# TAMUparametric/PPOPT

Measured on NVIDIA B200. Metric: candidate active sets/sec, higher is better.
Workload: dtype f64

## Files before the change

ppopt_b200/csrc/api.cu:

```cuda
#include <cstdio>
#include <cstdlib>
#include <cstring>
#include <mutex>
#include <string>
#include <vector>

#include "../../include/ppgpu.h"
#include "common.cuh"
#include "host_math.hpp"
#include "launch.h"

using namespace ppgpu;

static thread_local std::string g_err;

struct ppgpu_program {
    ReducedProgram host;
    DevProgram dev;
    int device = 0;
    int sm_count = 0;
    std::vector<void*> allocs;
    unsigned long long* d_counters = nullptr;
    unsigned long long* d_queue = nullptr;
    int queue_slot = 0;
// ... 291 lines not shown
    if (stages & 2) {
        ProfScope ps(p, st, 1);
        e = launch_k2(p->dev, d_masks, n, d_status, next_queue(p, st), p->d_counters, p->sm_count, st);
        if (e != cudaSuccess) return fail("K2 feasibility", e);
        p->launches++;
        if (p->dev.warm_count) {
            if ((e = launch_clear_bits(d_status, n, PPG_ST_PRE, st)) != cudaSuccess) return fail("status clean-up", e);
            p->launches++;
        }
    }
    if (stages & 4) {
        ProfScope ps(p, st, 2);
        if (p->dev.is_qp && p->dev.use_gram) {
            e = launch_k34(p->dev, d_masks, n, k_act, d_status, next_queue(p, st), p->d_counters, p->sm_count, st);
            if (k_act >= 1 && k_act <= 8) p->launches++;
        } else {
            e = launch_mark_general(p->dev, n, k_act, d_status, st);
        }
        if (e != cudaSuccess) return fail("K3/K4 optimality screen", e);
        p->launches++;
    }
    return 0;
}

int ppgpu_level_eval(ppgpu_program* p, const uint64_t* d_masks, int64_t n, int32_t k_act, uint8_t* d_status,
                     int32_t stages, ppgpu_stream stream) {
    return ppgpu_level_eval_w(p, d_masks, n, k_act, d_status, stages, nullptr, nullptr, 0, nullptr, nullptr, stream);
}

int ppgpu_level_eval_w(ppgpu_program* p, const uint64_t* d_masks, int64_t n, int32_t k_act, uint8_t* d_status,
                       int32_t stages, uint64_t* d_witness, const uint64_t* d_parent_feas, int64_t parent_nf,
                       const void* d_parent_ws, const uint64_t* d_parent_wit, ppgpu_stream stream) {
    if (!p) return fail_msg("null argument");
    if (n <= 0) return 0;
    WitnessIo wio;
    wio.parent_feas = d_parent_feas; wio.parent_nf = parent_nf; wio.parent_ws = d_parent_ws; wio.parent_wit = d_parent_wit;
    const bool walk = (stages & 2) && !(stages & 8) && k_act >= 1 && p->dev.wk_ok && p->k2w_min >= 0 && n >= p->k2w_min;
    const long long chunk = walk ? walk_chunk() : level_chunk();
    for (int64_t off = 0; off < n; off += chunk) {
        const int64_t nn = n - off < chunk ? n - off : chunk;
        wio.out = d_witness ? d_witness + (size_t)off * PPGPU_WITNESS_SLOTS * p->dev.W : nullptr;
        const int rc = level_eval_chunk(p, d_masks + (size_t)off * p->dev.W, nn, k_act, d_status + off, stages,
                                        (cudaStream_t)stream, wio);
        if (rc) return rc;
    }
    return 0;
}

size_t ppgpu_scan_workspace_bytes(int64_t n) { return scan_workspace_bytes(n); }
size_t ppgpu_select_workspace_bytes(int64_t n) { return select_workspace_bytes(n); }

int ppgpu_level_select(ppgpu_program* p, const uint8_t* d_status, int64_t n, uint8_t bits, uint8_t value,
                       int64_t* d_idx_out, int64_t* h_count, void* d_ws, size_t ws_bytes, ppgpu_stream stream) {
    if (!p || !h_count) return fail_msg("null argument");
    *h_count = 0;
    if (n <= 0) return 0;
    cudaStream_t st = (cudaStream_t)stream;
    if (ws_bytes < select_workspace_bytes(n)) return fail_msg("workspace too small");
    long long* d_count = (long long*)d_ws + (select_workspace_bytes(n) / sizeof(long long) - 1);
    cudaError_t e;
    {
        ProfScope ps(p, st, 6);
        e = select_indices(d_status, n, bits, value, (long long*)d_idx_out, d_count, d_ws, ws_bytes - sizeof(long long), st);
    }
    if (e != cudaSuccess) return fail("select", e);
    p->launches += 5;
    long long cnt = 0;
    e = cudaMemcpyAsync(&cnt, d_count, sizeof(long long), cudaMemcpyDeviceToHost, st);
    if (e == cudaSuccess) e = cudaStreamSynchronize(st);
    if (e != cudaSuccess) return fail("select count", e);
    *h_count = cnt;
    return 0;
}

int ppgpu_regions_emit(ppgpu_program* p, const uint64_t* d_masks, const int64_t* d_sel, int64_t n_sel, int32_t k_act,
                       double* d_laws, double* d_rows, int32_t* d_flags, double* d_info, uint8_t* d_status,
                       ppgpu_stream stream) {
    if (!p) return fail_msg("null argument");
    if (n_sel <= 0) return 0;
    cudaError_t e;
    {
        ProfScope ps(p, (cudaStream_t)stream, 3);
        e = launch_k5(p->dev, d_masks, (const long long*)d_sel, n_sel, k_act, d_laws, d_rows, d_flags, d_info, d_status,
                      p->d_counters, p->sm_count, (cudaStream_t)stream);
    }
    if (e != cudaSuccess) return fail("K5 emit", e);
    p->launches++;
    return 0;
}

int ppgpu_children_count(ppgpu_program* p, const uint64_t* d_masks, const int64_t* d_feas_idx, int64_t nf,
                         int32_t k_act, uint64_t* d_feas_masks, uint64_t* d_survive, int64_t* d_offsets,
                         int64_t* h_total, void* d_ws, size_t ws_bytes, ppgpu_stream stream) {
    if (!p || !h_total) return fail_msg("null argument");
    *h_total = 0;
    if (nf <= 0) return 0;
    cudaStream_t st = (cudaStream_t)stream;
    cudaError_t e;
    {
        ProfScope ps(p, st, 4);
        e = children_count(p->dev, d_masks, (const long long*)d_feas_idx, nf, k_act, d_feas_masks, d_survive,
                           (long long*)d_offsets, d_ws, ws_bytes, p->d_counters, st);
    }
    if (e != cudaSuccess) return fail("K6 count", e);
    p->launches += 12;
    long long tot = 0, disorder = 0;
    e = cudaMemcpyAsync(&tot, (long long*)d_offsets + nf, sizeof(long long), cudaMemcpyDeviceToHost, st);
    if (e == cudaSuccess) e = cudaMemcpyAsync(&disorder, children_order_flag(d_ws, nf), sizeof(long long), cudaMemcpyDeviceToHost, st);
    if (e == cudaSuccess) e = cudaStreamSynchronize(st);
    if (e != cudaSuccess) return fail("K6 total", e);
    if (disorder) return fail_msg("K6: the feasible parents are not one level's sets in lexicographic order");
    *h_total = tot;
    return 0;
}

int ppgpu_children_prepare(ppgpu_program* p, const uint64_t* d_masks, const int64_t* d_feas_idx, int64_t nf,
                           uint64_t* d_feas_masks, void* d_ws, size_t ws_bytes, ppgpu_stream stream) {
    if (!p) return fail_msg("null argument");
    if (nf <= 0) return 0;
    cudaError_t e;
    {
        ProfScope ps(p, (cudaStream_t)stream, 4);
        e = children_prepare(p->dev, d_masks, (const long long*)d_feas_idx, nf, d_feas_masks, d_ws, ws_bytes, (cudaStream_t)stream);
    }
    if (e != cudaSuccess) return fail("K6 prepare", e);
    p->launches += 8;
    return 0;
}

int ppgpu_children_count_range(ppgpu_program* p, const uint64_t* d_feas_masks, int64_t nf, int32_t k_act,
                               uint64_t* d_survive, int64_t* d_counts, int64_t p_lo, int64_t p_hi, void* d_ws,
                               size_t ws_bytes, ppgpu_stream stream) {
    if (!p) return fail_msg("null argument");
    if (p_lo < 0 || p_hi > nf || p_lo > p_hi) return fail_msg("parent range outside [0, nf]");
    if (nf <= 0 || p_hi == p_lo) return 0;
    if (ws_bytes < scan_workspace_bytes(nf)) return fail_msg("workspace too small");
    cudaError_t e;
    {
        ProfScope ps(p, (cudaStream_t)stream, 4);
        e = children_count_range(p->dev, d_feas_masks, nf, k_act, d_survive, (long long*)d_counts, p_lo, p_hi, d_ws,
                                 p->d_counters, (cudaStream_t)stream);
    }
    if (e != cudaSuccess) return fail("K6 count", e);
    p->launches++;
    return 0;
}

int ppgpu_children_scan(ppgpu_program* p, int64_t* d_counts_to_offsets, int64_t nf, int64_t* h_total, void* d_ws,
                        size_t ws_bytes, ppgpu_stream stream) {
    if (!p || !h_total) return fail_msg("null argument");
    *h_total = 0;
    if (nf <= 0) return 0;
    if (ws_bytes < scan_workspace_bytes(nf)) return fail_msg("workspace too small");
    cudaStream_t st = (cudaStream_t)stream;
    cudaError_t e;
    {
        ProfScope ps(p, st, 4);
        e = children_scan((long long*)d_counts_to_offsets, nf, d_ws, st);
    }
    if (e != cudaSuccess) return fail("K6 scan", e);
    p->launches += 2;
    long long tot = 0, disorder = 0;
    e = cudaMemcpyAsync(&tot, (long long*)d_counts_to_offsets + nf, sizeof(long long), cudaMemcpyDeviceToHost, st);
    if (e == cudaSuccess) e = cudaMemcpyAsync(&disorder, children_order_flag(d_ws, nf), sizeof(long long), cudaMemcpyDeviceToHost, st);
    if (e == cudaSuccess) e = cudaStreamSynchronize(st);
    if (e != cudaSuccess) return fail("K6 total", e);
    if (disorder) return fail_msg("K6: the feasible parents are not one level's sets in lexicographic order");
    *h_total = tot;
    return 0;
}
// ... 128 lines not shown
```

ppopt_b200/csrc/k34c_compact.cu:

```cuda
#include "common.cuh"
#include "launch.h"
#include "lp_core.cuh"

#include <cstdlib>

namespace ppgpu {

struct K4cOut { int code; double beta; int pivots; long long work; };

__device__ __forceinline__ double k4c_rcp(double x) {
    double r;
    asm("rcp.approx.ftz.f64 %0, %1;" : "=d"(r) : "d"(x));
    r = r * fma(-x, r, 2.0);
    return r * fma(-x, r, 2.0);
}

__device__ __noinline__ K4cOut k4c_solve(double* __restrict__ Tab, unsigned char* __restrict__ flag, int* __restrict__ bvar,
                                         double* __restrict__ alpha, int* __restrict__ kind, int* __restrict__ nbv,
                                         double* __restrict__ prow, int m, int t, int lds, double thr, int lane) {
    const int nc = t + 1;
    const int ld = nc + 1;
    K4cOut out; out.code = PPG_LP_OPTIMAL; out.beta = -CUDART_INF; out.pivots = 0; out.work = 0;
    int live = 0;
    #pragma unroll 1
    for (int i = lane; i < m; i += 32) { bvar[i] = ld + i; live += flag[i] ? 1 : 0; }
    live = __reduce_add_sync(PPG_FULL, live);
    #pragma unroll 1
    for (int c = lane; c < ld; c += 32) { alpha[c] = 0.0; kind[c] = (c >= 1) ? 1 : 0; nbv[c] = c; }
    __syncwarp();
    double beta = 0.0;
    int degen = 0; bool bland = false;
    const int cap = 50 * (m + nc) + 200;
    for (int it = 0;; ++it) {
        int j, l; double dir = 1.0;
        if (it == 0) {
            double mn = CUDART_INF; int r0 = 0x7fffffff;
            #pragma unroll 1
            for (int i = lane; i < m; i += 32)
                if (flag[i]) { const double v = Tab[(size_t)i * lds]; if (v < mn) { mn = v; r0 = i; } }
            warp_argmin(mn, r0);
            if (r0 == 0x7fffffff) { out.code = PPG_LP_UNBOUNDED; out.beta = CUDART_INF; return out; }
            j = nc; l = r0;
            if (lane == 0) alpha[nc] = -1.0;
            __syncwarp();
        } else {
            out.beta = beta;
            if (beta >= thr) { out.code = PPG_LP_EARLY; return out; }
            if (it > cap) { out.code = PPG_LP_ITERLIM; return out; }
            double sc = 0.0; int key = 0x7fffffff, jc = 0x7fffffff;
            #pragma unroll 1
            for (int c = 1 + lane; c < ld; c += 32) {
                const double a = alpha[c];
                const double s2 = kind[c] == 1 ? fabs(a) : (kind[c] == 2 ? -a : 0.0);
                if (s2 > PPG_OPT_TOL) {
                    if (!bland) { if (s2 > sc) { sc = s2; jc = c; } }
                    else if (nbv[c] < key) { key = nbv[c]; jc = c; sc = s2; }
                }
            }
            if (!__any_sync(PPG_FULL, jc != 0x7fffffff)) { out.code = PPG_LP_OPTIMAL; return out; }
            if (!bland) {
                const double ws = warp_max_nonneg(sc);
                j = __reduce_min_sync(PPG_FULL, (jc != 0x7fffffff && sc == ws) ? jc : 0x7fffffff);
            } else {
                const int wk = __reduce_min_sync(PPG_FULL, key);
                j = __reduce_min_sync(PPG_FULL, key == wk ? jc : 0x7fffffff);
            }
            const double aj = alpha[j];
            const bool entering_free = kind[j] == 1;
            dir = (entering_free && aj > 0.0) ? -1.0 : 1.0;
            double hb = CUDART_INF;
            #pragma unroll 1
            for (int i = lane; i < m; i += 32) {
                if (!flag[i]) continue;
                const double cv = dir * Tab[(size_t)i * lds + j];
                if (cv > PPG_TINY) {
                    const double rhs = fmax(Tab[(size_t)i * lds], 0.0);
                    hb = fmin(hb, (rhs + PPG_HARRIS) * k4c_rcp(cv));
                }
            }
            hb = warp_min_nonneg(hb);
            if (hb == CUDART_INF) { out.code = PPG_LP_UNBOUNDED; out.beta = CUDART_INF; return out; }
            double lp = 0.0, lr = CUDART_INF; int lrow = 0x7fffffff, lb = 0x7fffffff;
            #pragma unroll 1
            for (int i = lane; i < m; i += 32) {
                if (!flag[i]) continue;
                const double cv = dir * Tab[(size_t)i * lds + j];
                if (cv > PPG_TINY) {
                    const double rat = fmax(Tab[(size_t)i * lds], 0.0) * k4c_rcp(cv);
                    if (rat <= hb) {
                        const bool better = bland ? (bvar[i] < lb) : (cv > lp);
                        if (better) { lp = cv; lrow = i; lb = bvar[i]; lr = rat; }
                    }
                }
            }
            if (bland) {
                const int wb = __reduce_min_sync(PPG_FULL, lb);
                l = __reduce_min_sync(PPG_FULL, lb == wb ? lrow : 0x7fffffff);
            } else {
                const double wp = warp_max_nonneg(lp);
                l = __reduce_min_sync(PPG_FULL, (lrow != 0x7fffffff && lp == wp) ? lrow : 0x7fffffff);
            }
            if (l == 0x7fffffff) { out.code = PPG_LP_UNBOUNDED; out.beta = CUDART_INF; return out; }
            const double gr = __shfl_sync(PPG_FULL, lr, l & 31);
            if (gr <= PPG_DEGEN_STEP) { if (++degen > PPG_BLAND_AFTER) bland = true; } else degen = 0;
        }
        const bool entering_free = kind[j] == 1;
        double* Tl = Tab + (size_t)l * lds;
        const double inv = k4c_rcp(Tl[j]);
        __syncwarp();
        #pragma unroll 1
        for (int c = lane; c < ld; c += 32) prow[c] = (c == j) ? 0.0 : Tl[c] * inv;
        __syncwarp();
        const double aj = alpha[j];
        #pragma unroll 1
        for (int i = lane; i < m; i += 32) {
            if (!flag[i] || i == l) continue;
            double* Ti = Tab + (size_t)i * lds;
            const double col = Ti[j];
            if (col != 0.0) {
                #pragma unroll 1
                for (int c = 0; c < ld; ++c) Ti[c] = fma(-col, prow[c], Ti[c]);
                Ti[j] = -col * inv;
            }
            if (Ti[0] < 0.0 && Ti[0] > -1e-9) Ti[0] = 0.0;
        }
        __syncwarp();
        beta = fma(-aj, prow[0], beta);
        #pragma unroll 1
        for (int c = 1 + lane; c < ld; c += 32) alpha[c] = (c == j) ? -aj * inv : fma(-aj, prow[c], alpha[c]);
        #pragma unroll 1
        for (int c = lane; c < ld; c += 32) Tl[c] = (c == j) ? inv : prow[c];
        out.pivots++; out.work += (long long)live * (nc + 1);
        if (lane == 0) {
            const int leave_var = bvar[l], enter_var = nbv[j];
            kind[j] = 2; nbv[j] = leave_var;
            if (entering_free) flag[l] = 0; else bvar[l] = enter_var;
        }
        if (entering_free) live--;
        __syncwarp();
    }
}

__global__ void __launch_bounds__(128)
k34c_kernel(DevProgram P, const uint64_t* __restrict__ masks, long long n, int k_act, uint8_t* __restrict__ status,
            unsigned long long* __restrict__ queue, unsigned long long* __restrict__ counters, int use_pre, int warp_bytes,
            int lds) {
    extern __shared__ unsigned char k34c_smem[];
    const int warp = threadIdx.x >> 5, lane = threadIdx.x & 31;
    const int t = P.t, t1 = P.t + 1, mi = P.mi, W = P.W, k = k_act, m = P.R0;
    unsigned char* base = k34c_smem + (size_t)warp * warp_bytes;
    double* Tab = reinterpret_cast<double*>(base); base += (size_t)m * lds * 8;
    double* S = reinterpret_cast<double*>(base); base += (size_t)k * k * 8;
    double* Lam = reinterpret_cast<double*>(base); base += (size_t)k * t1 * 8;
    double* alpha = reinterpret_cast<double*>(base); base += (size_t)lds * 8;
    double* prow = reinterpret_cast<double*>(base); base += (size_t)lds * 8;
    int* act = reinterpret_cast<int*>(base); base += (size_t)((k + 1) & ~1) * 4;
    int* bvar = reinterpret_cast<int*>(base); base += (size_t)((m + 1) & ~1) * 4;
    int* kind = reinterpret_cast<int*>(base); base += (size_t)((lds + 1) & ~1) * 4;
    int* nbv = reinterpret_cast<int*>(base); base += (size_t)((lds + 1) & ~1) * 4;
    unsigned char* flag = base;
    unsigned long long n_lp = 0, n_piv = 0, n_work = 0, n_num = 0;
    const long long nblocks = (n + 31) / 32;
    for (;;) {
        unsigned long long v = 0;
        if (lane == 0) v = atomicAdd(queue, 1ull);
        const long long item = (long long)__shfl_sync(PPG_FULL, v, 0);
        if (item >= nblocks) break;
        const long long c0 = item * 32 + lane;
        const uint8_t sb = c0 < n ? status[c0] : 0;
        unsigned todo = __ballot_sync(PPG_FULL, (sb & PPG_ST_FEAS) && (!use_pre || (sb & PPG_ST_PRE)));
        while (todo) {
            const int src = __ffs((int)todo) - 1;
            todo &= todo - 1u;
            const long long idx = item * 32 + src;
            uint8_t st = (uint8_t)__shfl_sync(PPG_FULL, (int)sb, src);
            if (use_pre) st &= (uint8_t)~PPG_ST_PRE;
            const uint64_t* mk = masks + idx * W;
            __syncwarp();
            #pragma unroll 1
            for (int j = lane; j < k; j += 32) act[j] = mask_nth(mk, W, j);
            __syncwarp();
            #pragma unroll 1
            for (int e = lane; e < k * k; e += 32) {
                const int a = e / k, b2 = e - a * k;
                S[e] = __ldg(P.G + (size_t)act[a] * mi + act[b2]);
            }
            __syncwarp();
            bool pd = true;
            #pragma unroll 1
            for (int j = 0; j < k; ++j) {
                const double d = S[j * k + j];
                if (!(d > 0.0)) { pd = false; break; }
                const double sd = sqrt(d);
                __syncwarp();
                #pragma unroll 1
                for (int i = j + 1 + lane; i < k; i += 32) S[i * k + j] /= sd;
                if (lane == 0) S[j * k + j] = sd;
                __syncwarp();
                #pragma unroll 1
                for (int i = j + 1 + lane; i < k; i += 32) {
                    const double lij = S[i * k + j];
                    #pragma unroll 1
                    for (int c = j + 1; c <= i; ++c) S[i * k + c] = fma(-lij, S[c * k + j], S[i * k + c]);
                }
                __syncwarp();
            }
            bool pass = false, numeric = false, thin = false;
            if (!pd) {
                numeric = true;
            } else {
                if (lane < t1) {
                    #pragma unroll 1
                    for (int i = 0; i < k; ++i) {
                        double s = -__ldg(P.V + (size_t)act[i] * t1 + lane);
                        #pragma unroll 1
                        for (int j = 0; j < i; ++j) s = fma(-S[i * k + j], Lam[j * t1 + lane], s);
                        Lam[i * t1 + lane] = s / S[i * k + i];
                    }
                    #pragma unroll 1
                    for (int i = k - 1; i >= 0; --i) {
                        double s = Lam[i * t1 + lane];
                        #pragma unroll 1
                        for (int j = i + 1; j < k; ++j) s = fma(-S[j * k + i], Lam[j * t1 + lane], s);
                        Lam[i * t1 + lane] = s / S[i * k + i];
                    }
                }
                __syncwarp();
                bool reject = false;
                #pragma unroll 1
                for (int j = lane; j < k; j += 32) {
                    double ub = Lam[j * t1], mx = 0.0, mag = fabs(Lam[j * t1]);
                    #pragma unroll 1
                    for (int c = 0; c < t; ++c) {
                        const double a = Lam[j * t1 + 1 + c];
                        const double lo = __ldg(P.th_lo + c), hi = __ldg(P.th_hi + c);
                        mx = fmax(mx, fabs(a));
                        if (a != 0.0) { const double term = fmax(a * lo, a * hi); ub += term; mag += fabs(term); }
                    }
                    if (mx > PPG_ZERO_ROW) { if (ub < -1e-9 * fmax(1.0, mag)) reject = true; }
                    else if (mx <= PPG_ZERO_ROW && Lam[j * t1] < -PPG_FEAS_TOL) reject = true;
                }
                if (__any_sync(PPG_FULL, reject)) {
                    if (use_pre && lane == 0) status[idx] = st;
                    continue;
                }
                bool zero_viol = false;
                double lo1 = -CUDART_INF, hi1 = CUDART_INF;
                #pragma unroll 1
                for (int row = lane; row < m; row += 32) {
                    double* T = Tab + (size_t)row * lds;
                    if (row < mi) {
                        if (mask_test(mk, row)) {
                            const int pos = mask_rank(mk, row);
                            T[0] = Lam[pos * t1];
                            #pragma unroll 1
                            for (int c = 1; c < t1; ++c) T[c] = -Lam[pos * t1 + c];
                        } else {
// ... 4 lines not shown
                                const double g = __ldg(P.G + (size_t)act[a] * mi + row);
                                #pragma unroll 1
                                for (int c = 0; c < t1; ++c) T[c] = fma(g, Lam[a * t1 + c], T[c]);
                            }
                            #pragma unroll 1
                            for (int c = 1; c < t1; ++c) T[c] = -T[c];
                        }
                    } else {
                        const int o = row - mi;
                        T[0] = __ldg(P.b_t + o);
                        #pragma unroll 1
                        for (int c = 1; c < t1; ++c) T[c] = __ldg(P.A_t + (size_t)o * t + c - 1);
                    }
                    double mx = 0.0, nn = 0.0;
                    #pragma unroll 1
                    for (int c = 1; c < t1; ++c) { mx = fmax(mx, fabs(T[c])); nn = fma(T[c], T[c], nn); }
                    unsigned char fl = 0;
                    if (!(mx <= PPG_ZERO_ROW)) {
                        const double inv = 1.0 / sqrt(nn);
                        #pragma unroll 1
                        for (int c = 0; c < t1; ++c) T[c] *= inv;
                        T[t1] = 1.0;
                        fl = 1;
                        if (t == 1) { const double q = T[0] / T[1]; if (T[1] > 0.0) hi1 = fmin(hi1, q); else lo1 = fmax(lo1, q); }
                    } else if (T[0] < -PPG_FEAS_TOL) {
                        zero_viol = true;
                    }
                    flag[row] = fl;
                }
                __syncwarp();
                if (!__any_sync(PPG_FULL, zero_viol)) {
                    if (t == 1) {
#pragma unroll
                        for (int o = 16; o > 0; o >>= 1) {
                            lo1 = fmax(lo1, shfl_xor_d(lo1, o));
                            hi1 = fmin(hi1, shfl_xor_d(hi1, o));
                        }
                        pass = (lo1 + 0.5 * PPG_WIDTH_1D <= hi1);
                    } else {
                        const K4cOut res = k4c_solve(Tab, flag, bvar, alpha, kind, nbv, prow, m, t, lds, PPG_RADIUS_SCREEN, lane);
                        pass = res.code == PPG_LP_EARLY || (res.code == PPG_LP_OPTIMAL && res.beta >= PPG_RADIUS_SCREEN);
                        thin = res.code == PPG_LP_OPTIMAL && !pass && res.beta >= -PPG_RADIUS_BAND;
                        if (res.code == PPG_LP_ITERLIM) numeric = true;
                        n_lp++; n_piv += res.pivots; n_work += (unsigned long long)res.work;
                    }
                }
            }
            if (lane == 0) {
                uint8_t s2 = st;
                if (pass) s2 |= PPG_ST_OPT;
                if (thin) s2 |= PPG_ST_THIN;
                if (numeric) { s2 |= PPG_ST_NUMERIC; n_num++; }
                if (s2 != st || use_pre) status[idx] = s2;
            }
        }
    }
    if (lane == 0 && (n_lp || n_num)) {
        atomicAdd(&counters[CNT_K4_LPS], n_lp);
        atomicAdd(&counters[CNT_K4_PIVOTS], n_piv);
        atomicAdd(&counters[CNT_K4_WORK], n_work);
        if (n_num) atomicAdd(&counters[CNT_NUMERIC], n_num);
    }
}

cudaError_t launch_k34_compact(const DevProgram& P, const uint64_t* masks, long long n, int k_act, uint8_t* status,
                               unsigned long long* queue, unsigned long long* counters, int sm_count, cudaStream_t st,
                               int use_pre, bool* handled) {
    *handled = false;
    static const int on = getenv("PPGPU_K34_COMPACT") ? atoi(getenv("PPGPU_K34_COMPACT")) : 1;
    if (!on) return cudaSuccess;
    constexpr int WPC = 4;
    const int m = P.R0, t1 = P.t + 1, ld = P.t + 2, lds = ld | 1, k = k_act;
    size_t wb = (size_t)m * lds * 8 + (size_t)k * k * 8 + (size_t)k * t1 * 8 + (size_t)2 * lds * 8 +
                (size_t)(((k + 1) & ~1) + ((m + 1) & ~1) + 2 * ((lds + 1) & ~1)) * 4 + (size_t)m;
    wb = (wb + 15) & ~(size_t)15;
    const size_t smem = wb * WPC;
    if (smem > 200 * 1024) return cudaSuccess;
    cudaError_t e = allow_max_smem(k34c_kernel);
    if (e != cudaSuccess) return e;
    int occ = 0;
    e = cudaOccupancyMaxActiveBlocksPerMultiprocessor(&occ, k34c_kernel, 32 * WPC, smem);
    if (e != cudaSuccess) return e;
    if (occ < 1) occ = 1;
    long long grid = (long long)sm_count * occ;
    const long long need = (n + 32 * WPC - 1) / (32 * WPC);
    if (grid > need) grid = need;
    if (grid < 1) grid = 1;
    k34c_kernel<<<(unsigned)grid, 32 * WPC, smem, st>>>(P, masks, n, k_act, status, queue, counters, use_pre, (int)wb, lds);
    *handled = true;
    return cudaGetLastError();
}

__global__ void __launch_bounds__(128)
cheb_batch_kernel(const double* __restrict__ rows, const long long* __restrict__ row_off, long long n_poly, int t,
                  double* __restrict__ radius, int* __restrict__ code, int warp_bytes, int lds, int max_rows) {
    extern __shared__ unsigned char cheb_smem[];
    const int warp = threadIdx.x >> 5, lane = threadIdx.x & 31, t1 = t + 1;
    unsigned char* base = cheb_smem + (size_t)warp * warp_bytes;
    double* Tab = reinterpret_cast<double*>(base); base += (size_t)max_rows * lds * 8;
    double* alpha = reinterpret_cast<double*>(base); base += (size_t)lds * 8;
    double* prow = reinterpret_cast<double*>(base); base += (size_t)lds * 8;
    int* bvar = reinterpret_cast<int*>(base); base += (size_t)((max_rows + 1) & ~1) * 4;
    int* kind = reinterpret_cast<int*>(base); base += (size_t)((lds + 1) & ~1) * 4;
    int* nbv = reinterpret_cast<int*>(base); base += (size_t)((lds + 1) & ~1) * 4;
    unsigned char* flag = base;
    for (long long p = (long long)blockIdx.x * (blockDim.x >> 5) + warp; p < n_poly; p += (long long)gridDim.x * (blockDim.x >> 5)) {
        const long long r0 = row_off[p];
        const int m = (int)(row_off[p + 1] - r0);
        bool bad = false;
        __syncwarp();
#pragma unroll 1
        for (int i = lane; i < m; i += 32) {
            const double* src = rows + (size_t)(r0 + i) * t1;
            double* T = Tab + (size_t)i * lds;
            double nn = 0.0;
            T[0] = src[0];
#pragma unroll 1
            for (int c = 1; c < t1; ++c) { T[c] = src[c]; nn = fma(src[c], src[c], nn); }
            T[t1] = sqrt(nn);
            flag[i] = nn > 0.0 ? 1 : 0;
            if (!(nn > 0.0) && src[0] < 0.0) bad = true;
        }
        __syncwarp();
        K4cOut res; res.code = PPG_LP_INFEAS_EQ; res.beta = -CUDART_INF;
        if (!__any_sync(PPG_FULL, bad) && m > 0)
            res = k4c_solve(Tab, flag, bvar, alpha, kind, nbv, prow, m, t, lds, CUDART_INF, lane);
        if (lane == 0) { radius[p] = res.beta; code[p] = res.code; }
    }
}

cudaError_t launch_cheb_batch(const double* rows, const long long* row_off, long long n_poly, int t, int max_rows,
                              double* radius, int* code, int sm_count, cudaStream_t st) {
    constexpr int WPC = 4;
    const int ld = t + 2, lds = ld | 1;
    size_t wb = (size_t)max_rows * lds * 8 + (size_t)2 * lds * 8 + (size_t)(((max_rows + 1) & ~1) + 2 * ((lds + 1) & ~1)) * 4 +
                (size_t)max_rows;
    wb = (wb + 15) & ~(size_t)15;
    const size_t smem = wb * WPC;
    if (smem > 200 * 1024) return cudaErrorInvalidValue;
    cudaError_t e = allow_max_smem(cheb_batch_kernel);
    if (e != cudaSuccess) return e;
    long long grid = (n_poly + WPC - 1) / WPC;
    if (grid > (long long)sm_count * 4) grid = (long long)sm_count * 4;
    if (grid < 1) return cudaSuccess;
    cheb_batch_kernel<<<(unsigned)grid, 32 * WPC, smem, st>>>(rows, row_off, n_poly, t, radius, code, (int)wb, lds, max_rows);
    return cudaGetLastError();
}

}
```

ppopt_b200/csrc/k5_emit.cu:

```cuda
#include "common.cuh"
#include "launch.h"
#include "lp_core.cuh"

namespace ppgpu {

constexpr int K5_WARPS = 4;
constexpr int K5_THREADS = K5_WARPS * 32;

template <int RPT, int DC>
__global__ void __launch_bounds__(K5_THREADS)
k5_emit_kernel(DevProgram P, const uint64_t* __restrict__ masks, const long long* __restrict__ sel, long long n_sel,
               int k_act, double* __restrict__ laws_out, double* __restrict__ rows_out, int32_t* __restrict__ flags_out,
               double* __restrict__ info_out, uint8_t* __restrict__ status, unsigned long long* __restrict__ counters) {
    typedef LpCore<1, RPT, DC> Core;
    extern __shared__ double dyn_smem[];
    __shared__ typename Core::Shared sh_all[K5_WARPS];
    __shared__ double red_v[K5_WARPS];
    __shared__ int red_i[K5_WARPS];
    __shared__ double s_info[4];
    __shared__ int s_ok;
    __shared__ int s_full;
    __shared__ int s_thin;
    const int tid = threadIdx.x, warp = tid >> 5, lane = tid & 31;
    const int n = P.n, t = P.t, t1 = P.t + 1, m = P.m, ne = P.ne, mi = P.mi, R0 = P.R0, W = P.W;
    const int k = ne + k_act, N = n + k, ld = N + t1;
    double* M = dyn_smem;
    double* rows = M + (size_t)N * ld;
    int* flags = reinterpret_cast<int*>(rows + (size_t)R0 * t1);
    int* actf = flags + R0;
    int* keptf = actf + k;
    unsigned long long n_lp = 0, n_piv = 0, n_work = 0;

    for (long long si = blockIdx.x; si < n_sel; si += gridDim.x) {
        const long long idx = sel[si];
        const uint64_t* mk = masks + idx * W;
        __syncthreads();
        for (int j = tid; j < k; j += K5_THREADS) actf[j] = j < ne ? j : ne + mask_nth(mk, W, j - ne);
        if (tid == 0) { s_ok = 1; s_full = 0; s_thin = 0; s_info[0] = 0.0; s_info[1] = -CUDART_INF; s_info[2] = -CUDART_INF; s_info[3] = CUDART_INF; }
        __syncthreads();
        for (int e = tid; e < N * ld; e += K5_THREADS) {
            const int r = e / ld, c = e - r * ld;
            double v = 0.0;
            if (r < k) {
                const int row = actf[r];
                if (c < n) v = __ldg(P.A + (size_t)row * n + c);
                else if (c == N) v = __ldg(P.b + row);
                else if (c > N) v = __ldg(P.F + (size_t)row * t + (c - N - 1));
            } else {
                const int i = r - k;
                if (c < n) v = __ldg(P.Q + (size_t)i * n + c);
                else if (c < N) v = __ldg(P.A + (size_t)actf[c - n] * n + i);
                else if (c == N) v = -__ldg(P.c + i);
                else v = -__ldg(P.H + (size_t)i * t + (c - N - 1));
            }
            M[e] = v;
        }
        __syncthreads();
        for (int col = 0; col < N; ++col) {
            double best = -1.0; int p = 0x7fffffff;
            for (int i = col + tid; i < N; i += K5_THREADS) {
                const double a = fabs(M[(size_t)i * ld + col]);
                if (a > best) { best = a; p = i; }
            }
            warp_argmax(best, p);
            if (lane == 0) { red_v[warp] = best; red_i[warp] = p; }
            __syncthreads();
            best = red_v[0]; p = red_i[0];
#pragma unroll
            for (int w = 1; w < K5_WARPS; ++w)
                if (red_v[w] > best || (red_v[w] == best && red_i[w] < p)) { best = red_v[w]; p = red_i[w]; }
            if (!(best > 0.0) || !isfinite(best)) { if (tid == 0) s_ok = 0; __syncthreads(); break; }
            if (p != col) {
                for (int c = tid; c < ld; c += K5_THREADS) {
                    const double a = M[(size_t)p * ld + c];
                    M[(size_t)p * ld + c] = M[(size_t)col * ld + c];
                    M[(size_t)col * ld + c] = a;
                }
            }
            __syncthreads();
            const double inv = 1.0 / M[(size_t)col * ld + col];
            __syncthreads();
            for (int i = col + 1 + tid; i < N; i += K5_THREADS) M[(size_t)i * ld + col] *= inv;
            __syncthreads();
            const int tw = ld - col - 1, th = N - col - 1;
            for (int e = tid; e < tw * th; e += K5_THREADS) {
                const int i = col + 1 + e / tw, c = col + 1 + e % tw;
                M[(size_t)i * ld + c] = fma(-M[(size_t)i * ld + col], M[(size_t)col * ld + c], M[(size_t)i * ld + c]);
            }
            __syncthreads();
        }
        __syncthreads();
        const bool singular = s_ok == 0;
// ... 77 lines not shown
            if (warp == 0) {
                if (t == 1) {
                    double lo = -CUDART_INF, hi = CUDART_INF;
                    for (int r = lane; r < R0; r += 32)
                        if (flags[r] & 1) {
                            const double q = rows[(size_t)r * 2] / rows[(size_t)r * 2 + 1];
                            if (rows[(size_t)r * 2 + 1] > 0.0) hi = fmin(hi, q); else lo = fmax(lo, q);
                        }
#pragma unroll
                    for (int o = 16; o > 0; o >>= 1) {
                        lo = fmax(lo, shfl_xor_d(lo, o));
                        hi = fmin(hi, shfl_xor_d(hi, o));
                    }
                    if (lane == 0) {
                        s_info[1] = 0.5 * (hi - lo); s_info[2] = lo; s_info[3] = hi;
                        s_full = (lo + PPG_WIDTH_1D <= hi) ? 1 : 0;
                    }
                } else {
                    double rad_lo = -CUDART_INF, rad_hi = -CUDART_INF;
                    int code = PPG_LP_OPTIMAL;
                    for (int attempt = 0; attempt < 2; ++attempt) {
                        double T[RPT][DC];
                        int rflag[RPT], bv[RPT];
                        static_for<RPT>([&](auto RR) {
                            constexpr int rr = decltype(RR)::value;
                            const int row = rr * 32 + lane;
                            const bool on = row < R0 && (flags[row] & 1);
#pragma unroll
                            for (int c = 0; c < DC; ++c) T[rr][c] = (on && c < t1) ? rows[(size_t)row * t1 + c] : ((on && c == t1) ? 1.0 : 0.0);
                            rflag[rr] = on ? 1 : 0;
                            bv[rr] = 0;
                        });
                        const double thr = attempt == 0 ? PPG_RADIUS + PPG_RADIUS_BAND : CUDART_INF;
                        LpOut res = Core::solve(sh_all[0], T, rflag, R0, t1, thr, true, lane, true, &bv);
                        n_lp++; n_piv += res.pivots; n_work += (unsigned long long)res.work;
                        code = res.code;
                        rad_hi = res.beta;
                        if (code != PPG_LP_EARLY && code != PPG_LP_OPTIMAL) break;
                        double* th = &sh_all[0].P[0][0][0];
                        __syncwarp();
                        if (lane < t) th[lane] = 0.0;
                        __syncwarp();
                        static_for<RPT>([&](auto RR) {
                            constexpr int rr = decltype(RR)::value;
                            if (rflag[rr] == 3) {
                                const int c = bv[rr] < 0 ? -bv[rr] : bv[rr];
                                if (c >= 1 && c <= t) th[c - 1] = bv[rr] < 0 ? -T[rr][0] : T[rr][0];
                            }
                        });
                        __syncwarp();
                        double lo = CUDART_INF;
                        for (int r = lane; r < R0; r += 32)
                            if (flags[r] & 1) {
                                double sl = rows[(size_t)r * t1];
                                for (int c = 0; c < t; ++c) sl = fma(-rows[(size_t)r * t1 + 1 + c], th[c], sl);
                                lo = fmin(lo, sl);
                            }
#pragma unroll
                        for (int o = 16; o > 0; o >>= 1) lo = fmin(lo, shfl_xor_d(lo, o));
                        rad_lo = lo;
                        __syncwarp();
                        if (code == PPG_LP_OPTIMAL || rad_lo > PPG_RADIUS + PPG_RADIUS_BAND) break;
                    }
                    const bool solved = code == PPG_LP_EARLY || code == PPG_LP_OPTIMAL;
                    const bool ok = solved && rad_lo > PPG_RADIUS;
                    if (lane == 0) {
                        s_info[1] = solved ? rad_lo : rad_hi;
                        s_full = ok ? 1 : 0;
                        s_thin = (solved && rad_hi >= -PPG_RADIUS_BAND && rad_lo <= PPG_RADIUS + PPG_RADIUS_BAND) ? 1 : 0;
                    }
                }
            }
            __syncthreads();
            region = s_full != 0;
        }
        if (region) {
            if (t == 1) {
                const double lo = s_info[2], hi = s_info[3];
                for (int r = tid; r < R0; r += K5_THREADS)
                    if (flags[r] & 1) {
                        const double q = rows[(size_t)r * 2] / rows[(size_t)r * 2 + 1];
                        if (lo <= q && q <= hi) keptf[r] = 1;
                    }
            } else {
                for (int a = warp; a < R0; a += K5_WARPS) {
                    if (!(flags[a] & 1)) continue;
                    double T[RPT][DC];
                    int rflag[RPT];
                    static_for<RPT>([&](auto RR) {
                        constexpr int rr = decltype(RR)::value;
                        const int row = rr * 32 + lane;
                        const bool on = row < R0 && (flags[row] & 1);
#pragma unroll
                        for (int c = 0; c < DC; ++c)
                            T[rr][c] = (on && c < t1) ? rows[(size_t)row * t1 + c] : ((on && c == t1 && row != a) ? 1.0 : 0.0);
                        rflag[rr] = on ? (row == a ? 2 : 1) : 0;
                    });
                    LpOut res = Core::solve(sh_all[warp], T, rflag, R0, t1, -PPG_REDUND_TOL, false, lane);
                    n_lp++; n_piv += res.pivots; n_work += (unsigned long long)res.work;
                    const bool feas = res.code == PPG_LP_EARLY || res.code == PPG_LP_UNBOUNDED ||
                                      (res.code == PPG_LP_OPTIMAL && res.beta >= -PPG_REDUND_TOL);
                    if (lane == 0 && feas) keptf[a] = 1;
                }
            }
            __syncthreads();
            for (int r = tid; r < R0; r += K5_THREADS) if (keptf[r]) flags[r] |= 2;
            __syncthreads();
            if (t != 1) {
                for (int i = tid; i < R0; i += K5_THREADS) {
                    bool dup = false;
                    if ((flags[i] & 3) == 3) {
                        for (int j = 0; j < i && !dup; ++j) {
                            if ((flags[j] & 3) != 3) continue;
                            bool same = true;
                            for (int c = 0; c < t1 && same; ++c) same = rows[(size_t)i * t1 + c] == rows[(size_t)j * t1 + c];
                            dup = same;
                        }
                    }
                    keptf[i] = dup ? 1 : 0;
                }
                __syncthreads();
                for (int r = tid; r < R0; r += K5_THREADS) if (keptf[r]) flags[r] |= 4;
            }
            __syncthreads();
        }
        for (int e = tid; e < R0 * t1; e += K5_THREADS) rows_out[(size_t)si * R0 * t1 + e] = singular ? 0.0 : rows[e];
        for (int r = tid; r < R0; r += K5_THREADS) flags_out[(size_t)si * R0 + r] = singular ? 0 : flags[r];
        if (tid == 0) {
            info_out[si * 4 + 0] = region ? 1.0 : (singular ? -1.0 : 0.0);
            info_out[si * 4 + 1] = s_info[1];
            info_out[si * 4 + 2] = s_info[2];
            info_out[si * 4 + 3] = s_info[3];
            uint8_t st = status[idx];
            if (region) st |= PPG_ST_REGION;
            if (s_thin && !singular) st |= PPG_ST_THIN;
            if (singular) st |= PPG_ST_NUMERIC;
            status[idx] = st;
        }
    }
    if (lane == 0 && n_lp) {
        atomicAdd(&counters[CNT_K5_LPS], n_lp);
        atomicAdd(&counters[CNT_K5_PIVOTS], n_piv);
        atomicAdd(&counters[CNT_K5_WORK], n_work);
    }
}

template <int RPT, int DC>
static cudaError_t launch_k5_t(const DevProgram& P, const uint64_t* masks, const long long* idx, long long n_sel, int k_act,
                               double* laws, double* rows, int32_t* flags, double* info, uint8_t* status,
                               unsigned long long* counters, int sm_count, cudaStream_t st) {
    auto kern = k5_emit_kernel<RPT, DC>;
    const int k = P.ne + k_act, N = P.n + k, ld = N + P.t + 1;
    const size_t smem = ((size_t)N * ld + (size_t)P.R0 * (P.t + 1)) * sizeof(double) + (size_t)(2 * P.R0 + k + 2) * sizeof(int);
    if (smem > 200 * 1024) return cudaErrorInvalidValue;
    cudaError_t e;
    if ((e = fit_smem(kern, smem)) != cudaSuccess) return e;
    long long grid = n_sel;
    const long long cap = (long long)sm_count * 8;
    if (grid > cap) grid = cap;
    if (grid < 1) return cudaSuccess;
    kern<<<(unsigned)grid, K5_THREADS, smem, st>>>(P, masks, idx, n_sel, k_act, laws, rows, flags, info, status, counters);
    return cudaGetLastError();
}

#define K5_RPT_SWITCH(DCV)                                                                                                            \
    if (P.R0 <= 32) return launch_k5_t<1, DCV>(P, masks, idx, n_sel, k_act, laws, rows, flags, info, status, counters, sm_count, st);  \
    if (P.R0 <= 64) return launch_k5_t<2, DCV>(P, masks, idx, n_sel, k_act, laws, rows, flags, info, status, counters, sm_count, st);  \
    if (P.R0 <= 128) return launch_k5_t<4, DCV>(P, masks, idx, n_sel, k_act, laws, rows, flags, info, status, counters, sm_count, st); \
    if (P.R0 <= 256) return launch_k5_t<8, DCV>(P, masks, idx, n_sel, k_act, laws, rows, flags, info, status, counters, sm_count, st); \
    return cudaErrorInvalidValue;

cudaError_t launch_k5(const DevProgram& P, const uint64_t* masks, const long long* idx, long long n_sel, int k_act,
                      double* laws, double* rows, int32_t* flags, double* info, uint8_t* status,
                      unsigned long long* counters, int sm_count, cudaStream_t st) {
    if (P.t + 2 <= 8) { K5_RPT_SWITCH(8) }
    if (P.t + 2 <= 16) { K5_RPT_SWITCH(16) }
    return cudaErrorInvalidValue;
}

}
```

ppopt_b200/csrc/launch.h:

```cpp
#pragma once
#include <cuda_runtime.h>
#include <stdint.h>

#include "common.cuh"

namespace ppgpu {

template <class K>
inline cudaError_t allow_max_smem(K kern) {
    int dev = 0, lim = 0;
    cudaError_t e = cudaGetDevice(&dev);
    if (e == cudaSuccess) e = cudaDeviceGetAttribute(&lim, cudaDevAttrMaxSharedMemoryPerBlockOptin, dev);
    if (e != cudaSuccess) return e;
    cudaFuncAttributes fa;
    if ((e = cudaFuncGetAttributes(&fa, kern)) != cudaSuccess) return e;
    return cudaFuncSetAttribute(kern, cudaFuncAttributeMaxDynamicSharedMemorySize, lim - (int)fa.sharedSizeBytes);
}

template <class K>
inline cudaError_t fit_smem(K kern, size_t dyn) {
    cudaFuncAttributes fa;
    const cudaError_t e = cudaFuncGetAttributes(&fa, kern);
    if (e != cudaSuccess) return e;
    return fa.sharedSizeBytes + dyn > 48 * 1024 ? allow_max_smem(kern) : cudaSuccess;
}

int k2_pad_columns(int ncols_with_rhs);

cudaError_t launch_k1(const DevProgram& P, const uint64_t* masks, long long n, int k_act, uint8_t* status,
                      unsigned long long* counters, int sm_count, cudaStream_t st);
cudaError_t launch_k2(const DevProgram& P, const uint64_t* masks, long long n, uint8_t* status,
                      unsigned long long* queue, unsigned long long* counters, int sm_count, cudaStream_t st);
cudaError_t launch_k2a(const DevProgram& P, const uint64_t* masks, long long n, int k_act, uint8_t* status,
                       unsigned long long* queue, unsigned long long* counters, int max_iter, int sm_count, cudaStream_t st);
cudaError_t launch_k2a_prefix(const DevProgram& P, const uint64_t* masks, long long n, int k_act, uint8_t* status,
                              unsigned long long* queue, unsigned long long* counters, int max_iter, int sm_count,
                              cudaStream_t st, bool* handled);
cudaError_t launch_k2w(const DevProgram& P, const uint64_t* masks, long long n, int k_act, uint8_t* status,
                       unsigned long long* queue, unsigned long long* counters, int sm_count, cudaStream_t st, bool* handled,
                       uint64_t* witness, int* order_scratch);
size_t k2w_order_scratch_ints(long long n);
cudaError_t launch_inherit(const DevProgram& P, const uint64_t* masks, long long n, uint8_t* status, uint64_t* witness_out,
                           const uint64_t* parent_feas, long long parent_nf, const void* parent_ws, const uint64_t* parent_wit,
                           unsigned long long* counters, cudaStream_t st);
cudaError_t launch_k34(const DevProgram& P, const uint64_t* masks, long long n, int k_act, uint8_t* status,
                       unsigned long long* queue, unsigned long long* counters, int sm_count, cudaStream_t st);
cudaError_t launch_k34_compact(const DevProgram& P, const uint64_t* masks, long long n, int k_act, uint8_t* status,
                               unsigned long long* queue, unsigned long long* counters, int sm_count, cudaStream_t st,
                               int use_pre, bool* handled);
cudaError_t launch_mark_general(const DevProgram& P, long long n, int k_act, uint8_t* status, cudaStream_t st);

cudaError_t launch_k5(const DevProgram& P, const uint64_t* masks, const long long* idx, long long n_sel, int k_act,
                      double* laws, double* rows, int32_t* flags, double* info, uint8_t* status,
                      unsigned long long* counters, int sm_count, cudaStream_t st);

size_t scan_workspace_bytes(long long n);
size_t select_workspace_bytes(long long n);
const long long* children_order_flag(const void* ws, long long nf);
cudaError_t select_indices(const uint8_t* status, long long n, uint8_t bits, uint8_t value, long long* idx_out,
                           long long* d_count, void* ws, size_t ws_bytes, cudaStream_t st);
cudaError_t root_level(const DevProgram& P, uint64_t* masks, long long* d_count, cudaStream_t st);
cudaError_t children_count(const DevProgram& P, const uint64_t* masks, const long long* feas_idx, long long nf,
                           int k_act, uint64_t* feas_masks, uint64_t* survive, long long* offsets, void* ws,
                           size_t ws_bytes, unsigned long long* counters, cudaStream_t st);
cudaError_t children_prepare(const DevProgram& P, const uint64_t* masks, const long long* feas_idx, long long nf,
                             uint64_t* feas_masks, void* ws, size_t ws_bytes, cudaStream_t st);
cudaError_t children_count_range(const DevProgram& P, const uint64_t* feas_masks, long long nf, int k_act, uint64_t* survive,
                                 long long* counts, long long p_lo, long long p_hi, void* ws, unsigned long long* counters,
                                 cudaStream_t st);
cudaError_t children_scan(long long* counts_to_offsets, long long nf, void* ws, cudaStream_t st);
cudaError_t children_write(const DevProgram& P, const uint64_t* feas_masks, const uint64_t* survive,
                           const long long* offsets, long long nf, uint64_t* children, cudaStream_t st);

cudaError_t launch_locate(const double* theta, long long n_points, int t, const double* rows, const long long* row_off,
                          long long n_regions, const double* laws, int n_x, int use_tol, double tol, int overlap,
                          const double* Qm, const double* Hm, const double* cv, int* region_out, double* x_out, int sm_count,
                          cudaStream_t st);

cudaError_t launch_cheb_batch(const double* rows, const long long* row_off, long long n_poly, int t, int max_rows,
                              double* radius, int* code, int sm_count, cudaStream_t st);
cudaError_t launch_theta_qp(const DevProgram& P, const double* theta, long long n_points, uint8_t* status, double* x,
                            double* dual, uint64_t* mask, int* iters, int sm_count, cudaStream_t st);
cudaError_t launch_theta_lp(const DevProgram& P, const double* theta, long long n_points, uint8_t* status, double* x,
                            double* dual, uint64_t* mask, int* iters, int sm_count, cudaStream_t st);
cudaError_t launch_clear_bits(uint8_t* status, long long n, uint8_t bits, cudaStream_t st);

cudaError_t measure_fp64_peak(int iters, double* tflops, cudaStream_t st);

}
```

Measured before the change: 357.2 million.

## Split K5 redundancy LPs into separate work-queue kernel and adapt K34c item size

```diff
diff --git a/ppopt_b200/csrc/api.cu b/ppopt_b200/csrc/api.cu
--- a/ppopt_b200/csrc/api.cu
+++ b/ppopt_b200/csrc/api.cu
@@ -397,10 +397,10 @@
     {
         ProfScope ps(p, (cudaStream_t)stream, 3);
         e = launch_k5(p->dev, d_masks, (const long long*)d_sel, n_sel, k_act, d_laws, d_rows, d_flags, d_info, d_status,
-                      p->d_counters, p->sm_count, (cudaStream_t)stream);
+                      next_queue(p, (cudaStream_t)stream), p->d_counters, p->sm_count, (cudaStream_t)stream);
     }
     if (e != cudaSuccess) return fail("K5 emit", e);
-    p->launches++;
+    p->launches += k5_launches(p->dev.t);
     return 0;
 }
 
diff --git a/ppopt_b200/csrc/k34c_compact.cu b/ppopt_b200/csrc/k34c_compact.cu
--- a/ppopt_b200/csrc/k34c_compact.cu
+++ b/ppopt_b200/csrc/k34c_compact.cu
@@ -2,6 +2,7 @@
 #include "launch.h"
 #include "lp_core.cuh"
 
+#include <algorithm>
 #include <cstdlib>
 
 namespace ppgpu {
@@ -144,7 +145,7 @@
 __global__ void __launch_bounds__(128)
 k34c_kernel(DevProgram P, const uint64_t* __restrict__ masks, long long n, int k_act, uint8_t* __restrict__ status,
             unsigned long long* __restrict__ queue, unsigned long long* __restrict__ counters, int use_pre, int warp_bytes,
-            int lds) {
+            int lds, int per_item) {
     extern __shared__ unsigned char k34c_smem[];
     const int warp = threadIdx.x >> 5, lane = threadIdx.x & 31;
     const int t = P.t, t1 = P.t + 1, mi = P.mi, W = P.W, k = k_act, m = P.R0;
@@ -160,19 +161,19 @@
     int* nbv = reinterpret_cast<int*>(base); base += (size_t)((lds + 1) & ~1) * 4;
     unsigned char* flag = base;
     unsigned long long n_lp = 0, n_piv = 0, n_work = 0, n_num = 0;
-    const long long nblocks = (n + 31) / 32;
+    const long long nblocks = (n + per_item - 1) / per_item;
     for (;;) {
         unsigned long long v = 0;
         if (lane == 0) v = atomicAdd(queue, 1ull);
         const long long item = (long long)__shfl_sync(PPG_FULL, v, 0);
         if (item >= nblocks) break;
-        const long long c0 = item * 32 + lane;
-        const uint8_t sb = c0 < n ? status[c0] : 0;
+        const long long c0 = item * per_item + lane;
+        const uint8_t sb = (lane < per_item && c0 < n) ? status[c0] : 0;
         unsigned todo = __ballot_sync(PPG_FULL, (sb & PPG_ST_FEAS) && (!use_pre || (sb & PPG_ST_PRE)));
         while (todo) {
             const int src = __ffs((int)todo) - 1;
             todo &= todo - 1u;
-            const long long idx = item * 32 + src;
+            const long long idx = item * per_item + src;
             uint8_t st = (uint8_t)__shfl_sync(PPG_FULL, (int)sb, src);
             if (use_pre) st &= (uint8_t)~PPG_ST_PRE;
             const uint64_t* mk = masks + idx * W;
@@ -343,11 +344,15 @@
     e = cudaOccupancyMaxActiveBlocksPerMultiprocessor(&occ, k34c_kernel, 32 * WPC, smem);
     if (e != cudaSuccess) return e;
     if (occ < 1) occ = 1;
+    const long long warps = (long long)sm_count * occ * WPC;
+    const int per_item = (int)std::min<long long>(32, std::max<long long>(1, (n + warps - 1) / warps));
+    const long long items = (n + per_item - 1) / per_item;
     long long grid = (long long)sm_count * occ;
-    const long long need = (n + 32 * WPC - 1) / (32 * WPC);
+    const long long need = (items + WPC - 1) / WPC;
     if (grid > need) grid = need;
     if (grid < 1) grid = 1;
-    k34c_kernel<<<(unsigned)grid, 32 * WPC, smem, st>>>(P, masks, n, k_act, status, queue, counters, use_pre, (int)wb, lds);
+    k34c_kernel<<<(unsigned)grid, 32 * WPC, smem, st>>>(P, masks, n, k_act, status, queue, counters, use_pre, (int)wb, lds,
+                                                        per_item);
     *handled = true;
     return cudaGetLastError();
 }
diff --git a/ppopt_b200/csrc/k5_emit.cu b/ppopt_b200/csrc/k5_emit.cu
--- a/ppopt_b200/csrc/k5_emit.cu
+++ b/ppopt_b200/csrc/k5_emit.cu
@@ -1,3 +1,5 @@
+#include <cstdlib>
+
 #include "common.cuh"
 #include "launch.h"
 #include "lp_core.cuh"
@@ -7,7 +9,7 @@
 constexpr int K5_WARPS = 4;
 constexpr int K5_THREADS = K5_WARPS * 32;
 
-template <int RPT, int DC>
+template <int RPT, int DC, bool FUSED>
 __global__ void __launch_bounds__(K5_THREADS)
 k5_emit_kernel(DevProgram P, const uint64_t* __restrict__ masks, const long long* __restrict__ sel, long long n_sel,
                int k_act, double* __restrict__ laws_out, double* __restrict__ rows_out, int32_t* __restrict__ flags_out,
@@ -251,7 +253,7 @@
                         const double q = rows[(size_t)r * 2] / rows[(size_t)r * 2 + 1];
                         if (lo <= q && q <= hi) keptf[r] = 1;
                     }
-            } else {
+            } else if constexpr (FUSED) {
                 for (int a = warp; a < R0; a += K5_WARPS) {
                     if (!(flags[a] & 1)) continue;
                     double T[RPT][DC];
@@ -275,7 +277,7 @@
             __syncthreads();
             for (int r = tid; r < R0; r += K5_THREADS) if (keptf[r]) flags[r] |= 2;
             __syncthreads();
-            if (t != 1) {
+            if (FUSED && t != 1) {
                 for (int i = tid; i < R0; i += K5_THREADS) {
                     bool dup = false;
                     if ((flags[i] & 3) == 3) {
@@ -314,11 +316,107 @@
     }
 }
 
+constexpr int K5B_WARPS = 4;
+constexpr int K5B_CHUNK = 4;
+
+template <int RPT, int DC>
+constexpr int k5b_min_ctas() { return RPT * DC <= 16 ? 4 : (RPT * DC <= 32 ? 3 : (RPT * DC <= 64 ? 2 : 1)); }
+
+template <int RPT, int DC>
+__global__ void __launch_bounds__(K5B_WARPS * 32, k5b_min_ctas<RPT, DC>())
+k5_redund_kernel(int R0, int t1, long long n_sel, const double* __restrict__ rows_out, int32_t* flags_out,
+                 const double* __restrict__ info_out, unsigned long long* __restrict__ queue,
+                 unsigned long long* __restrict__ counters) {
+    typedef LpCore<1, RPT, DC> Core;
+    __shared__ typename Core::Shared sh_all[K5B_WARPS];
+    const int warp = threadIdx.x >> 5, lane = threadIdx.x & 31;
+    const long long n_pairs = n_sel * R0;
+    unsigned long long n_lp = 0, n_piv = 0, n_work = 0;
+    for (;;) {
+        unsigned long long v = 0;
+        if (lane == 0) v = atomicAdd(queue, (unsigned long long)K5B_CHUNK);
+        const long long base = (long long)__shfl_sync(PPG_FULL, v, 0);
+        if (base >= n_pairs) break;
+        bool live = false;
+        if (lane < K5B_CHUNK && base + lane < n_pairs) {
+            const long long pr = base + lane;
+            live = __ldg(info_out + (pr / R0) * 4) == 1.0 && (flags_out[pr] & 1);
+        }
+        unsigned todo = __ballot_sync(PPG_FULL, live);
+        while (todo) {
+            const int src = __ffs((int)todo) - 1;
+            todo &= todo - 1u;
+            const long long pr = base + src, si = pr / R0;
+            const int a = (int)(pr - si * R0);
+            const double* rows = rows_out + (size_t)si * R0 * t1;
+            const int32_t* flags = flags_out + (size_t)si * R0;
+            double T[RPT][DC];
+            int rflag[RPT];
+            static_for<RPT>([&](auto RR) {
+                constexpr int rr = decltype(RR)::value;
+                const int row = rr * 32 + lane;
+                const bool on = row < R0 && (flags[row] & 1);
+#pragma unroll
+                for (int c = 0; c < DC; ++c)
+                    T[rr][c] = (on && c < t1) ? __ldg(rows + (size_t)row * t1 + c) : ((on && c == t1 && row != a) ? 1.0 : 0.0);
+                rflag[rr] = on ? (row == a ? 2 : 1) : 0;
+            });
+            LpOut res = Core::solve(sh_all[warp], T, rflag, R0, t1, -PPG_REDUND_TOL, false, lane);
+            n_lp++; n_piv += res.pivots; n_work += (unsigned long long)res.work;
+            const bool feas = res.code == PPG_LP_EARLY || res.code == PPG_LP_UNBOUNDED ||
+                              (res.code == PPG_LP_OPTIMAL && res.beta >= -PPG_REDUND_TOL);
+            if (lane == 0 && feas) atomicOr(flags_out + pr, 2);
+        }
+    }
+    if (lane == 0 && n_lp) {
+        atomicAdd(&counters[CNT_K5_LPS], n_lp);
+        atomicAdd(&counters[CNT_K5_PIVOTS], n_piv);
+        atomicAdd(&counters[CNT_K5_WORK], n_work);
+    }
+}
+
+constexpr int K5C_WARPS = 4;
+
+__global__ void __launch_bounds__(K5C_WARPS * 32)
+k5_dedupe_kernel(int R0, int t1, long long n_sel, const double* __restrict__ rows_out, int32_t* __restrict__ flags_out,
+                 const double* __restrict__ info_out) {
+    const int lane = threadIdx.x & 31;
+    const long long nw = (long long)gridDim.x * K5C_WARPS;
+    for (long long si = (long long)blockIdx.x * K5C_WARPS + (threadIdx.x >> 5); si < n_sel; si += nw) {
+        if (__ldg(info_out + si * 4) != 1.0) continue;
+        const double* rows = rows_out + (size_t)si * R0 * t1;
+        int32_t* flags = flags_out + (size_t)si * R0;
+        unsigned dup = 0;
+        for (int i = lane, q = 0; i < R0; i += 32, ++q) {
+            if ((flags[i] & 3) != 3) continue;
+            bool d = false;
+            for (int j = 0; j < i && !d; ++j) {
+                if ((flags[j] & 3) != 3) continue;
+                bool same = true;
+                for (int c = 0; c < t1 && same; ++c) same = __ldg(rows + (size_t)i * t1 + c) == __ldg(rows + (size_t)j * t1 + c);
+                d = same;
+            }
+            if (d) dup |= 1u << q;
+        }
+        __syncwarp();
+        for (int i = lane, q = 0; i < R0; i += 32, ++q)
+            if ((dup >> q) & 1u) flags[i] |= 4;
+    }
+}
+
+static bool k5_fused() {
+    static const bool on = getenv("PPGPU_K5_FUSED") && atoi(getenv("PPGPU_K5_FUSED")) != 0;
+    return on;
+}
+
+int k5_launches(int t) { return k5_fused() || t == 1 ? 1 : 3; }
+
 template <int RPT, int DC>
 static cudaError_t launch_k5_t(const DevProgram& P, const uint64_t* masks, const long long* idx, long long n_sel, int k_act,
                                double* laws, double* rows, int32_t* flags, double* info, uint8_t* status,
-                               unsigned long long* counters, int sm_count, cudaStream_t st) {
-    auto kern = k5_emit_kernel<RPT, DC>;
+                               unsigned long long* queue, unsigned long long* counters, int sm_count, cudaStream_t st) {
+    const bool fused = k5_fused();
+    auto kern = fused ? k5_emit_kernel<RPT, DC, true> : k5_emit_kernel<RPT, DC, false>;
     const int k = P.ne + k_act, N = P.n + k, ld = N + P.t + 1;
     const size_t smem = ((size_t)N * ld + (size_t)P.R0 * (P.t + 1)) * sizeof(double) + (size_t)(2 * P.R0 + k + 2) * sizeof(int);
     if (smem > 200 * 1024) return cudaErrorInvalidValue;
@@ -329,19 +427,36 @@
     if (grid > cap) grid = cap;
     if (grid < 1) return cudaSuccess;
     kern<<<(unsigned)grid, K5_THREADS, smem, st>>>(P, masks, idx, n_sel, k_act, laws, rows, flags, info, status, counters);
+    if ((e = cudaGetLastError()) != cudaSuccess || fused || P.t == 1) return e;
+
+    auto kb = k5_redund_kernel<RPT, DC>;
+    if ((e = fit_smem(kb, 0)) != cudaSuccess) return e;
+    int occ = 0;
+    if ((e = cudaOccupancyMaxActiveBlocksPerMultiprocessor(&occ, kb, K5B_WARPS * 32, 0)) != cudaSuccess) return e;
+    if (occ < 1) occ = 1;
+    const long long items = (n_sel * P.R0 + K5B_CHUNK - 1) / K5B_CHUNK;
+    grid = (items + K5B_WARPS - 1) / K5B_WARPS;
+    if (grid > (long long)sm_count * occ) grid = (long long)sm_count * occ;
+    kb<<<(unsigned)grid, K5B_WARPS * 32, 0, st>>>(P.R0, P.t + 1, n_sel, rows, flags, info, queue, counters);
+    if ((e = cudaGetLastError()) != cudaSuccess) return e;
+
+    if ((e = fit_smem(k5_dedupe_kernel, 0)) != cudaSuccess) return e;
+    grid = (n_sel + K5C_WARPS - 1) / K5C_WARPS;
+    if (grid > (long long)sm_count * 16) grid = (long long)sm_count * 16;
+    k5_dedupe_kernel<<<(unsigned)grid, K5C_WARPS * 32, 0, st>>>(P.R0, P.t + 1, n_sel, rows, flags, info);
     return cudaGetLastError();
 }
 
-#define K5_RPT_SWITCH(DCV)                                                                                                            \
-    if (P.R0 <= 32) return launch_k5_t<1, DCV>(P, masks, idx, n_sel, k_act, laws, rows, flags, info, status, counters, sm_count, st);  \
-    if (P.R0 <= 64) return launch_k5_t<2, DCV>(P, masks, idx, n_sel, k_act, laws, rows, flags, info, status, counters, sm_count, st);  \
-    if (P.R0 <= 128) return launch_k5_t<4, DCV>(P, masks, idx, n_sel, k_act, laws, rows, flags, info, status, counters, sm_count, st); \
-    if (P.R0 <= 256) return launch_k5_t<8, DCV>(P, masks, idx, n_sel, k_act, laws, rows, flags, info, status, counters, sm_count, st); \
+#define K5_RPT_SWITCH(DCV)                                                                                                                   \
+    if (P.R0 <= 32) return launch_k5_t<1, DCV>(P, masks, idx, n_sel, k_act, laws, rows, flags, info, status, queue, counters, sm_count, st);  \
+    if (P.R0 <= 64) return launch_k5_t<2, DCV>(P, masks, idx, n_sel, k_act, laws, rows, flags, info, status, queue, counters, sm_count, st);  \
+    if (P.R0 <= 128) return launch_k5_t<4, DCV>(P, masks, idx, n_sel, k_act, laws, rows, flags, info, status, queue, counters, sm_count, st); \
+    if (P.R0 <= 256) return launch_k5_t<8, DCV>(P, masks, idx, n_sel, k_act, laws, rows, flags, info, status, queue, counters, sm_count, st); \
     return cudaErrorInvalidValue;
 
 cudaError_t launch_k5(const DevProgram& P, const uint64_t* masks, const long long* idx, long long n_sel, int k_act,
                       double* laws, double* rows, int32_t* flags, double* info, uint8_t* status,
-                      unsigned long long* counters, int sm_count, cudaStream_t st) {
+                      unsigned long long* queue, unsigned long long* counters, int sm_count, cudaStream_t st) {
     if (P.t + 2 <= 8) { K5_RPT_SWITCH(8) }
     if (P.t + 2 <= 16) { K5_RPT_SWITCH(16) }
     return cudaErrorInvalidValue;
diff --git a/ppopt_b200/csrc/launch.h b/ppopt_b200/csrc/launch.h
--- a/ppopt_b200/csrc/launch.h
+++ b/ppopt_b200/csrc/launch.h
@@ -52,7 +52,8 @@
 
 cudaError_t launch_k5(const DevProgram& P, const uint64_t* masks, const long long* idx, long long n_sel, int k_act,
                       double* laws, double* rows, int32_t* flags, double* info, uint8_t* status,
-                      unsigned long long* counters, int sm_count, cudaStream_t st);
+                      unsigned long long* queue, unsigned long long* counters, int sm_count, cudaStream_t st);
+int k5_launches(int t);
 
 size_t scan_workspace_bytes(long long n);
 size_t select_workspace_bytes(long long n);
```

Result: faster. 370.0 million, median of 6 (+3.6%).
